# WarmCongee/SDUMC

Hardware: AMD Instinct MI355X
Metric: train samples/sec at MOSEI feature shapes (two-stream forward + 6-term loss + backward + Adam) (higher is better)
Workload: dtype f32

## Files before the change

sdumc_amd/csrc/chain_cluster.hip:

```cpp
#include <atomic>
#include <mutex>

#include "chain_common.h"

namespace {

constexpr int CL = 4;
constexpr int OC = D / CL;
constexpr int HC = H / CL;
constexpr int PARTC = NWV * 7 * OC;
constexpr int SPIN_CAP = 400000;
static_assert(PARTC >= NWV * 2 * H, "tail layers");

template <int R> using FwdA = FwdALds<R, PARTC>;
template <int R> using FwdB = FwdBLds<R, PARTC, 3, 0>;
template <int R> using BwdB = BwdBLds<R, PARTC, 3>;
template <int R> using BwdA = BwdALds<R, PARTC, 3>;

struct Cl {
  uint32_t* arrive;
  uint32_t* depart;
  int32_t* err;
  uint32_t round;
  bool hold;
// ... 17 lines not shown
  for (int u = threadIdx.x; u < ROWS * q; u += NTHR) {
    const int r = u / q, c = u - r * q;
    st4(dst_lds + r * ld_dst + 4 * c, row0 + r < nrows ? ld4_dev(src + (int64_t)(row0 + r) * ld_src + 4 * c) : f32x4{0.f, 0.f, 0.f, 0.f});
  }
}

__device__ __forceinline__ void cl_sync(Cl& cl, int* s_bail) {
  if (cl.mode & 1u) __builtin_amdgcn_fence(__ATOMIC_RELEASE, "agent");
  __builtin_amdgcn_s_waitcnt(0);
  __syncthreads();
  if (threadIdx.x == 0 && !*s_bail) {
    if (!cl.hold) {
      if (cl.mode & 1u) __hip_atomic_fetch_add(cl.arrive, 1u, __ATOMIC_RELEASE, __HIP_MEMORY_SCOPE_AGENT);
      else __hip_atomic_fetch_add(cl.arrive, 1u, __ATOMIC_RELAXED, __HIP_MEMORY_SCOPE_AGENT);
    }
    const uint32_t want = (uint32_t)CL * (cl.round + 1u);
    int spins = 0;
    while (__hip_atomic_load(cl.arrive, __ATOMIC_RELAXED, __HIP_MEMORY_SCOPE_AGENT) < want) {
      if (++spins > SPIN_CAP) {
        *s_bail = 1;
        __hip_atomic_store(cl.err, 1, __ATOMIC_RELAXED, __HIP_MEMORY_SCOPE_AGENT);
        break;
      }
      __builtin_amdgcn_s_sleep(1);
    }
  }
  ++cl.round;
  __syncthreads();
  if (cl.mode & 1u) __builtin_amdgcn_fence(__ATOMIC_ACQUIRE, "agent");
}
__device__ __forceinline__ void cl_exit(Cl& cl) {
  if (threadIdx.x == 0) {
    const uint32_t n = __hip_atomic_fetch_add(cl.depart, 1u, __ATOMIC_RELAXED, __HIP_MEMORY_SCOPE_AGENT);
    if (n == (uint32_t)CL - 1u) {
      __hip_atomic_store(cl.arrive, 0u, __ATOMIC_RELAXED, __HIP_MEMORY_SCOPE_AGENT);
      __hip_atomic_store(cl.depart, 0u, __ATOMIC_RELAXED, __HIP_MEMORY_SCOPE_AGENT);
    }
  }
}

template <int I, int O, int RSv>
struct CGeom {
  static constexpr int OG = O / 4;
  static constexpr int S = 64 / OG;
  static constexpr int MW = NWV / RSv;
  static constexpr int UNITS = I / (4 * S);
  static constexpr int WAVES = UNITS >= MW ? MW : UNITS;
  static constexpr int IW = I / WAVES;
  static constexpr int ITER = IW / (4 * S);
  static constexpr int PRE = ITER >= 4 ? 4 : ITER;
  static_assert(O == 32 || O == 64, "slice width");
  static_assert(I % (4 * S * WAVES) == 0 && ITER >= 1, "k range must split evenly");
};
struct CRing {
  uint4 w[16];
};
template <int N, class F>
__device__ __forceinline__ void static_for(F&& f) {
  if constexpr (N > 0) {
    static_for<N - 1>(f);
    f(std::integral_constant<int, N - 1>{});
  }
}

template <int I, int O, int RSv, int SLOT>
__device__ __forceinline__ void cxm_load(CRing& ring, const float* mp, int j, int ldm) {
  using G = CGeom<I, O, RSv>;
  static_for<4>([&](auto ec) {
    constexpr int e = decltype(ec)::value;
    ring.w[SLOT * 4 + e] = *reinterpret_cast<const uint4*>(mp + (size_t)(j * 4 * G::S + e) * ldm);
  });
}

template <int I, int O, int RSv>
__device__ __forceinline__ void cxm_prefetch(CRing& ring, const float* __restrict__ M, int ldm) {
  using G = CGeom<I, O, RSv>;
  const int lane = threadIdx.x & 63, wg = (threadIdx.x >> 6) % G::MW;
  if (wg < G::WAVES) {
    const int sq = lane / G::OG, cg = lane % G::OG;
    const float* mp = M + (size_t)(wg * G::IW + 4 * sq) * ldm + 4 * cg;
    static_for<G::PRE>([&](auto dc) { cxm_load<I, O, RSv, decltype(dc)::value>(ring, mp, decltype(dc)::value, ldm); });
    static_for<16 - 4 * G::PRE>([&](auto kc) { ring.w[4 * G::PRE + decltype(kc)::value] = uint4{0u, 0u, 0u, 0u}; });
  }
}

template <int I, int O, int RSv>
__device__ __forceinline__ void cxm_selfcheck(const CRing& ring, const float* M, int ldm, uint32_t* dbg) {
  using G = CGeom<I, O, RSv>;
  const int lane = threadIdx.x & 63, wg = (threadIdx.x >> 6) % G::MW;
  if (wg < G::WAVES && dbg) {
    const int sq = lane / G::OG, cg = lane % G::OG;
    const float* mp = M + (size_t)(wg * G::IW + 4 * sq) * ldm + 4 * cg;
    static_for<G::PRE>([&](auto dc) {
      constexpr int sl = decltype(dc)::value;
      static_for<4>([&](auto ec) {
        constexpr int e = decltype(ec)::value;
        const uint32_t* ad = reinterpret_cast<const uint32_t*>(mp + (size_t)(sl * 4 * G::S + e) * ldm);
        const uint4 c = ring.w[sl * 4 + e];
        uint32_t b[4];
#pragma unroll
        for (int k = 0; k < 4; ++k) b[k] = __hip_atomic_load(ad + k, __ATOMIC_RELAXED, __HIP_MEMORY_SCOPE_AGENT);
        if (c.x != b[0] || c.y != b[1] || c.z != b[2] || c.w != b[3]) {
          const uint32_t idx = atomicAdd(dbg, 1u);
          if (idx < 20) {
            uint32_t* r = dbg + 8 + 12 * idx;
            r[0] = blockIdx.x; r[1] = threadIdx.x; r[2] = sl * 4 + e;
            r[3] = (uint32_t)(reinterpret_cast<uintptr_t>(ad) & 0xffffffffu);
            r[4] = c.x; r[5] = c.y; r[6] = c.z; r[7] = c.w; r[8] = b[0]; r[9] = b[1]; r[10] = b[2]; r[11] = b[3];
          }
        }
      });
    });
  }
}

constexpr int FOLD_MAXCHUNK = 32;
template <class T>
__device__ __forceinline__ T sel3v(T t0, T t1, T t2, int m) { return m == 0 ? t0 : (m == 1 ? t1 : t2); }
#define sel3(t, m) sel3v((t)[0], (t)[1], (t)[2], m)

struct ChunkItem {
  const float* src;
  int u, c0, nc;
};
template <int NU, class Desc>
__device__ __forceinline__ ChunkItem chunk_item(int u, int c0, Desc& desc) {
  ChunkItem it;
  it.u = u;
  it.c0 = c0;
  desc(min(u, NU - 1), it.src, it.nc);
  if (u >= NU) it.nc = -1;
  return it;
}
template <int STRIDE>
__device__ __forceinline__ void chunk_request(const ChunkItem& it, f32x4 (&pv)[8]) {
  static_for<8>([&](auto jc) {
    constexpr int j = decltype(jc)::value;
    if (it.c0 + j < it.nc) pv[j] = ld4(it.src + (size_t)(it.c0 + j) * STRIDE);
  });
}
template <int NU, int STRIDE, class Desc, class Acc, class Fin>
__device__ __forceinline__ void chunk_drain(ChunkItem cur, f32x4 (&pa)[8], Desc& desc, Acc&& acc, Fin&& fin) {
  f32x4 sum = {0.f, 0.f, 0.f, 0.f};
  while (cur.nc >= 0) {
    const bool more = cur.c0 + 8 < cur.nc;
    const ChunkItem nx = chunk_item<NU>(more ? cur.u : cur.u + NTHR, more ? cur.c0 + 8 : 0, desc);
    f32x4 pb[8];
    chunk_request<STRIDE>(nx, pb);
    if (cur.c0 == 0) sum = f32x4{0.f, 0.f, 0.f, 0.f};
    static_for<8>([&](auto jc) {
      constexpr int j = decltype(jc)::value;
      if (cur.c0 + j < cur.nc) acc(sum, pa[j], cur.u, cur.c0 + j);
    });
    if (!more) fin(cur.u, sum);
    cur = nx;
    static_for<8>([&](auto jc) { pa[decltype(jc)::value] = pb[decltype(jc)::value]; });
  }
}

template <int R, int NQT>
struct FoldHead {
  static constexpr int NS = 3 * R * NQT;
  static constexpr int NU = NS * (D / 4);
  static_assert(NS <= NTHR, "one statistics row per thread");
  float cm[8], cs[8];
  ChunkItem it;
// ... 154 lines not shown
}

template <int ROWS>
__device__ __forceinline__ void lds_selfcheck(const float* lds_rows, const float* src, int width, int row0, int nrows, uint32_t* dbg, int tag) {
  if (!dbg) return;
  const int q = width >> 2;
  for (int u = threadIdx.x; u < ROWS * q; u += NTHR) {
    const int r = u / q, c = u - r * q;
    if (row0 + r >= nrows) continue;
    const f32x4 l = ld4(lds_rows + r * width + 4 * c);
    const f32x4 g = ld4(src + (int64_t)(row0 + r) * width + 4 * c);
    if (__float_as_uint(l[0]) != __float_as_uint(g[0]) || __float_as_uint(l[1]) != __float_as_uint(g[1]) ||
        __float_as_uint(l[2]) != __float_as_uint(g[2]) || __float_as_uint(l[3]) != __float_as_uint(g[3])) {
      const uint32_t idx = atomicAdd(dbg, 1u);
      if (idx < 20) {
        uint32_t* rec = dbg + 8 + 12 * idx;
        rec[0] = blockIdx.x; rec[1] = threadIdx.x; rec[2] = (uint32_t)tag; rec[3] = (uint32_t)(r * width + 4 * c);
#pragma unroll
        for (int k = 0; k < 4; ++k) { rec[4 + k] = __float_as_uint(l[k]); rec[8 + k] = __float_as_uint(g[k]); }
      }
    }
  }
}

template <int ROWS, int I, int O, class Epi, class Hook>
__device__ __forceinline__ void cxm_run(CRing& ring, const float* in_lds, int ld_in, const float* __restrict__ M, int ldm, float* part,
                                        Epi&& epi, Hook&& hook) {
  constexpr int RSv = ROWS >= 14 ? 2 : 1;
  using G = CGeom<I, O, RSv>;
  constexpr int OG = G::OG, S = G::S, MW = G::MW, WAVES = G::WAVES, IW = G::IW, ITER = G::ITER;
  constexpr int RG = ROWS / RSv;
  static_assert(ROWS % RSv == 0 && RG <= 7, "rows per group");
  static_assert(RSv * WAVES * RG * O <= PARTC, "partial-sum area too small");
  const int tid = threadIdx.x, lane = tid & 63, wave = tid >> 6;
  const int grp = wave / MW, wg = wave % MW;
  const int sq = lane / OG, cg = lane % OG;
  f32x4 acc[RG];
#pragma unroll
  for (int r = 0; r < RG; ++r) acc[r] = f32x4{0.f, 0.f, 0.f, 0.f};
  if (wg < WAVES) {
    const int i0 = wg * IW + 4 * sq;
    const float* mp = M + (size_t)i0 * ldm + 4 * cg;
    const float* xin = in_lds + grp * RG * ld_in + i0;
    static_for<ITER>([&](auto jc) {
      constexpr int j = decltype(jc)::value, sl = (j % 4) * 4;
#pragma unroll
      for (int r = 0; r < RG; ++r) {
        const f32x4 x = ld4(xin + r * ld_in + j * 4 * S);
        static_for<4>([&](auto ec) {
          constexpr int e = decltype(ec)::value;
          const uint4 u = ring.w[sl + e];
          acc[r] += f32x4{__uint_as_float(u.x), __uint_as_float(u.y), __uint_as_float(u.z), __uint_as_float(u.w)} * x[e];
        });
      }
      __builtin_amdgcn_sched_barrier(0);
      if constexpr (j + 4 < ITER) cxm_load<I, O, RSv, j % 4>(ring, mp, j + 4, ldm);
    });
#pragma unroll
    for (int r = 0; r < RG; ++r)
#pragma unroll
      for (int c = 0; c < 4; ++c) {
        acc[r][c] += __shfl_xor(acc[r][c], 32, 64);
        acc[r][c] += __shfl_xor(acc[r][c], 16, 64);
        if constexpr (S == 8) acc[r][c] += __shfl_xor(acc[r][c], 8, 64);
      }
  }
  hook();
  if (wg < WAVES && sq == 0) {
#pragma unroll
    for (int r = 0; r < RG; ++r) st4(part + ((grp * WAVES + wg) * RG + r) * O + 4 * cg, acc[r]);
  }
  __syncthreads();
  for (int u = tid; u < ROWS * (O / 4); u += NTHR) {
    const int r = u / (O / 4), cq = u - r * (O / 4);
    const int g = r / RG, rr = r - g * RG;
    f32x4 v = ld4(part + ((g * WAVES) * RG + rr) * O + 4 * cq);
#pragma unroll
    for (int ww = 1; ww < WAVES; ++ww) v += ld4(part + ((g * WAVES + ww) * RG + rr) * O + 4 * cq);
    epi(r, 4 * cq, v);
  }
  __syncthreads();
}

#define TR(k) do { if (a.cl_trace && blockIdx.x == 0 && threadIdx.x == 0) a.cl_trace[k] = wall_clock64(); } while (0)

#define CL_PROLOGUE()                                                                                          \
  __shared__ int s_bail;                                                                                       \
  const int cluster = blockIdx.x % ncl, member = blockIdx.x / ncl;                                             \
  const int V = a.V, v0 = cluster * R, tid = threadIdx.x, lane = tid & 63, wave = tid >> 6;                    \
  const int coff = member * OC;                                                                                \
  Cl cl{a.cl_flags + cluster * 64, a.cl_flags + cluster * 64 + 32, a.cl_err, 0u, a.cl_test_hold == 1 && blockIdx.x == 0, (uint32_t)a.cl_mode};                              \
  if (tid == 0) s_bail = 0;                                                                                    \
  (void)lane; (void)wave

typedef float WT;
#define PF(I_, O_, ptr, ldm) cxm_prefetch<I_, O_, 1>(ring, ptr, ldm)
#define PF14(I_, O_, ptr, ldm) cxm_prefetch<I_, O_, 2>(ring, ptr, ldm)

template <int R>
__device__ __forceinline__ void chain_fwd_a_cl_body(const sdumc_chain_args a, const int ncl) {
  extern __shared__ __attribute__((aligned(16))) float sm[];
  using L = FwdA<R>;
  float *part = sm + L::part, *s_hpre = sm + L::hpre, *s_u1 = sm + L::u1, *s_u = sm + L::u, *s_att1 = sm + L::att1, *s_att2 = sm + L::att2,
        *s_qin = sm + L::qin, *s_q = sm + L::q, *s_bias = sm + L::bias;
  CL_PROLOGUE();
  TR(0);
  const int64_t VD = (int64_t)V * D;
  const bool fold = a.fra.part[0] != nullptr;
  FoldHead<R, 1> fh;
  FoldNorm<R, 1> fn;
  if (fold) {
    fold_request<R, 1>(fh, a.fra, v0, V);
    fold_norm_request<R, 1>(fn, a.fra, v0, V, member);
  }
  constexpr int NBIAS = (FWD_A_BIAS_UNITS + NTHR - 1) / NTHR;
  f32x4 bias[NBIAS];
  static_for<NBIAS>([&](auto kc) { bias[decltype(kc)::value] = ld4(fwd_a_bias_src(a, min(tid + decltype(kc)::value * NTHR, FWD_A_BIAS_UNITS - 1))); });
  const DropRT dbase = drop_resolve(a.drop);
  CRing ring;
  if (a.cl_mode & 2) __builtin_amdgcn_fence(__ATOMIC_ACQUIRE, "agent");
  if (a.cl_mode & 8)
    for (int i = 0; i < 8; ++i) __builtin_amdgcn_s_sleep(127);
  PF(D, OC, a.umlp0_w[0] + coff, D);
  if (a.cl_mode & 16) cxm_selfcheck<D, OC, 1>(ring, a.umlp0_w[0] + coff, D, a.cl_dbg);
  if (fold) fold_combine<R, 1>(fh, a.fra, a.hpre, s_hpre, s_qin, v0, V, member, dbase);
  else for (int m = 0; m < 3; ++m) load_rows<R>(s_hpre + m * R * D, a.hpre + m * VD, D, D, v0, V);
  static_for<NBIAS>([&](auto kc) {
    const int u = tid + decltype(kc)::value * NTHR;
    if (u < FWD_A_BIAS_UNITS) st4(s_bias + 4 * u, bias[decltype(kc)::value]);
  });
  __syncthreads();
  TR(11);
  if ((a.cl_mode & 64) && !a.fra.part[0])
    for (int m = 0; m < 3; ++m) lds_selfcheck<R>(s_hpre + m * R * D, a.hpre + m * VD, D, v0, V, a.cl_dbg, 10 + m);
#pragma unroll 1
  for (int m = 0; m < 3; ++m) {
    const DropRT dr = mkdrop_rt(dbase, 6 + 2 * m, 1, D);
    float* dst = a.u1 + m * VD + (int64_t)v0 * D;
    auto epi = [&](int r, int col, f32x4 v) {
      col += coff;
      if (v0 + r < V) st4_dev(dst + (int64_t)r * D + col, fwd_val(v, s_bias + m * D, col, true, dr, (uint32_t)(v0 + r)));
    };
    cxm_run<R, D, OC>(ring, s_hpre + m * R * D, D, a.umlp0_w[m] + coff, D, part, epi,
                                [&] { PF(D, OC, (m < 2 ? a.umlp0_w[m + 1] : a.umlp3_w[0]) + coff, D); });
  }
  if (fold) fold_norm_finish<R, 1>(fn, a.fra, s_qin, v0, V, member);
  TR(1);
  if ((a.cl_mode & 64) && !a.fra.part[0])
    for (int m = 0; m < 3; ++m) lds_selfcheck<R>(s_hpre + m * R * D, a.hpre + m * VD, D, v0, V, a.cl_dbg, 20 + m);
  cl_sync(cl, &s_bail);
  TR(2);
  for (int m = 0; m < 3; ++m) reload_rows<R>(s_u1 + m * R * D, D, a.u1 + m * VD, D, D, v0, V);
  __syncthreads();
#pragma unroll 1
  for (int m = 0; m < 3; ++m) {
    const DropRT dr = mkdrop_rt(dbase, 7 + 2 * m, 1, D);
    float* dst = a.u + (int64_t)v0 * 3 * D + m * D;
    auto epi = [&](int r, int col, f32x4 v) {
      col += coff;
      if (v0 + r < V) st4_dev(dst + (int64_t)r * 3 * D + col, fwd_val(v, s_bias + (3 + m) * D, col, true, dr, (uint32_t)(v0 + r)));
    };
    cxm_run<R, D, OC>(ring, s_u1 + m * R * D, D, a.umlp3_w[m] + coff, D, part, epi, [&] {
      if (m < 2) PF(D, OC, a.umlp3_w[m + 1] + coff, D);
      else PF(3 * D, OC, a.att0_w + coff, D);
    });
  }
  TR(3);
  cl_sync(cl, &s_bail);
  TR(4);
  reload_rows<R>(s_u, 3 * D, a.u, 3 * D, 3 * D, v0, V);
  __syncthreads();
  {
    const DropRT dr = mkdrop_rt(dbase, 12, 1, D);
    float* dst = a.att1 + (int64_t)v0 * D;
    auto epi = [&](int r, int col, f32x4 v) {
      col += coff;
      if (v0 + r < V) st4_dev(dst + (int64_t)r * D + col, fwd_val(v, s_bias + 6 * D, col, true, dr, (uint32_t)(v0 + r)));
    };
    cxm_run<R, 3 * D, OC>(ring, s_u, 3 * D, a.att0_w + coff, D, part, epi, [&] { PF(D, OC, a.att3_w + coff, D); });
  }
  TR(5);
  cl_sync(cl, &s_bail);
  TR(6);
  reload_rows<R>(s_att1, D, a.att1, D, D, v0, V);
  __syncthreads();
  {
    const DropRT dr = mkdrop_rt(dbase, 13, 1, D);
    float* dst = a.att2 + (int64_t)v0 * D;
    auto epi = [&](int r, int col, f32x4 v) {
      col += coff;
      if (v0 + r < V) st4_dev(dst + (int64_t)r * D + col, fwd_val(v, s_bias + 7 * D, col, true, dr, (uint32_t)(v0 + r)));
    };
    cxm_run<R, D, OC>(ring, s_att1, D, a.att3_w + coff, D, part, epi, [&] { PF(D, OC, a.query_w[0] + coff, D); });
  }
  TR(7);
  cl_sync(cl, &s_bail);
  TR(8);
  reload_rows<R>(s_att2, D, a.att2, D, D, v0, V);
  __syncthreads();
  fwd_a_alpha<L>(a, sm, v0, V, member == 0);
  fwd_a_fusion<L>(a, sm, v0, V, [member](int c) { return c / OC == member; });
#pragma unroll 1
  for (int i = 0; i < 7; ++i) {
    const DropRT dr = mkdrop_rt(dbase, 14 + i, 1, D);
    float* dst = a.q + (int64_t)v0 * NQ * D + i * D;
    float* th = (i == 5 && a.o_text_hidden) ? a.o_text_hidden + (int64_t)v0 * D : nullptr;
    auto epi = [&](int r, int col, f32x4 v) {
      col += coff;
      if (v0 + r < V) {
        const f32x4 y = fwd_val(v, s_bias + (8 + i) * D, col, true, dr, (uint32_t)(v0 + r));
        st4_dev(dst + (int64_t)r * NQ * D + col, y);
        if (th) st4(th + (int64_t)r * D + col, y);
      }
    };
    cxm_run<R, D, OC>(ring, s_qin + i * R * D, D, a.query_w[i] + coff, D, part, epi,
                                [&] { if (i < 6) PF(D, OC, a.query_w[i + 1] + coff, D); else PF14(D, OC, a.caq_w[0] + coff, D); });
  }
  TR(9);
  cl_sync(cl, &s_bail);
  TR(10);
  reload_rows<R>(s_q, NQ * D, a.q, NQ * D, NQ * D, v0, V);
  __syncthreads();
  cl_exit(cl);
#pragma unroll 1
  for (int m = 0; m < 3; ++m) {
    float* dst = a.qp + ((int64_t)m * V + v0) * NQ * D;
    auto epi = [&](int r, int col, f32x4 v) {
      col += coff;
      if (v0 + r / NQ < V) st4(dst + (int64_t)r * D + col, v + ld4(s_bias + (15 + m) * D + col));
    };
    cxm_run<NQ * R, D, OC>(ring, s_q, D, a.caq_w[m] + coff, D, part, epi, [&] { if (m < 2) PF14(D, OC, a.caq_w[m + 1] + coff, D); });
  }
  TR(31);
}
template <int R>
__global__ __launch_bounds__(NTHR) void chain_fwd_a_cl_kernel(const sdumc_chain_args a, const int ncl) { chain_fwd_a_cl_body<R>(a, ncl); }

template <int R>
__device__ __forceinline__ void chain_fwd_b_cl_body(const sdumc_chain_args a, const int ncl) {
  extern __shared__ __attribute__((aligned(16))) float sm[];
  using L = FwdB<R>;
  float *part = sm + L::part, *s_x = sm + L::x, *s_c = sm + L::c, *s_h = sm + L::h, *s_e1 = sm + L::e1, *s_e2 = sm + L::e2, *s_bias = sm + L::bias;
  CL_PROLOGUE();
  TR(0);
  const int64_t VQ = (int64_t)V * NQ;
  const int hoff = member * HC;
  const bool fold = a.ca.part[0] != nullptr;
  FoldHead<R, NQ> fh;
  FoldNorm<R, NQ> fn;
  if (fold) {
    fold_request<R, NQ>(fh, a.ca, v0, V);
    fold_norm_request<R, NQ>(fn, a.ca, v0, V, member);
  }
  static_assert(FWD_B_BIAS_UNITS <= NTHR, "one bias unit per thread");
  const f32x4 bias = ld4(fwd_b_bias_src(a, min(tid, FWD_B_BIAS_UNITS - 1)));
  const float al = alpha_request<R>(a.alpha, v0, V);
  const DropRT dbase = drop_resolve(a.drop);
  CRing ring;
  PF14(D, OC, a.cmlp0_w[0] + coff, D);
  if (fold) fold_combine<R, NQ>(fh, a.ca, a.ca_out, s_x, s_c, v0, V, member, dbase);
  else for (int m = 0; m < 3; ++m) load_rows<NQ * R>(s_x + m * NQ * R * D, a.ca_out + (int64_t)m * VQ * D, D, D, v0 * NQ, V * NQ);
  if (tid < FWD_B_BIAS_UNITS) st4(s_bias + 4 * tid, bias);
  alpha_store<R>(al, sm + L::alpha, v0, V);
  __syncthreads();
  TR(11);
#pragma unroll 1
  for (int m = 0; m < 3; ++m) {
    const DropRT dr = mkdrop_rt(dbase, 27 + 2 * m, NQ, D);
    float* dst = a.c1 + ((int64_t)m * VQ + (int64_t)v0 * NQ) * D;
    auto epi = [&](int r, int col, f32x4 v) {
      col += coff;
      if (v0 * NQ + r < V * NQ) st4_dev(dst + (int64_t)r * D + col, fwd_val(v, s_bias + m * D, col, true, dr, (uint32_t)(v0 * NQ + r)));
    };
    cxm_run<NQ * R, D, OC>(ring, s_x + m * NQ * R * D, D, a.cmlp0_w[m] + coff, D, part, epi, [&] {
      if (m < 2) PF14(D, OC, a.cmlp0_w[m + 1] + coff, D);
      else PF14(D, HC, a.cmlp3_w[0] + hoff, H);
    });
  }
  if (fold) fold_norm_finish<R, NQ>(fn, a.ca, s_c, v0, V, member);
  TR(1);
  cl_sync(cl, &s_bail);
  TR(2);
  for (int m = 0; m < 3; ++m) reload_rows<NQ * R>(s_x + m * NQ * R * D, D, a.c1 + (int64_t)m * VQ * D, D, D, v0 * NQ, V * NQ);
  __syncthreads();
#pragma unroll 1
  for (int m = 0; m < 3; ++m) {
    const DropRT dr = mkdrop_rt(dbase, 28 + 2 * m, NQ, H);
    float* dst = a.c + ((int64_t)m * VQ + (int64_t)v0 * NQ) * H;
    float* ct = (m == 1 && a.o_cross_text) ? a.o_cross_text + (int64_t)v0 * NQ * H : nullptr;
    auto epi = [&](int r, int col, f32x4 v) {
      col += hoff;
      if (v0 * NQ + r < V * NQ) {
        const f32x4 y = fwd_val(v, s_bias + 3 * D + m * H, col, true, dr, (uint32_t)(v0 * NQ + r));
        st4_dev(dst + (int64_t)r * H + col, y);
        if (ct) st4(ct + (int64_t)r * H + col, y);
      }
    };
    cxm_run<NQ * R, D, HC>(ring, s_x + m * NQ * R * D, D, a.cmlp3_w[m] + hoff, H, part, epi, [&] {
      if (m < 2) PF14(D, HC, a.cmlp3_w[m + 1] + hoff, H);
// ... 132 lines not shown
                                     [&] { if (m < 2) PF14(D, OC, a.cmlp0_w[m + 1] + coff, D); });
  }
  TR(31);
}
template <int R>
__global__ __launch_bounds__(NTHR) void chain_bwd_b_cl_kernel(const sdumc_chain_args a, const int ncl) { chain_bwd_b_cl_body<R>(a, ncl); }

template <int R>
__device__ __forceinline__ void chain_bwd_a_cl_body(const sdumc_chain_args a, const int ncl) {
  extern __shared__ __attribute__((aligned(16))) float sm[];
  using L = BwdA<R>;
  float *part = sm + L::part, *s_x = sm + L::x, *s_dq = sm + L::dq, *s_dqin = sm + L::dqin, *s_u = sm + L::u, *s_du = sm + L::du, *s_a2 = sm + L::a2,
        *s_a1 = sm + L::a1, *s_u1 = sm + L::u1;
  CL_PROLOGUE();
  TR(0);
  const int64_t VD = (int64_t)V * D, VQ = (int64_t)V * NQ;
  const float sc = a.relu_scale;
  const bool wr = member == 0;

  const bool slabs = a.dq_part[0] != nullptr;
  auto dq_desc = [&](int u, const float*& src, int& nc) {
    const int row = u / (D / 4), cq = u - row * (D / 4);
    const int mr = row / NQ, i = row - mr * NQ;
    const int m = mr / R, v = v0 + (mr - m * R);
    const int ncm = sel3(a.dq_nchunk, m);
    src = sel3(a.dq_part, m) + ((size_t)min(v, V - 1) * ncm * NQ + i) * D + 4 * cq;
    nc = v < V ? ncm : 0;
  };
  constexpr int NUX = 3 * R * NQ * (D / 4);
  ChunkItem it;
  f32x4 pa[8];
  RowsReg<NQ * R, D> x[3];
  if (slabs) {
    it = chunk_item<NUX>(tid, 0, dq_desc);
    chunk_request<NQ * D>(it, pa);
  } else {
    static_for<3>([&](auto mc) { rows_request(x[decltype(mc)::value], a.d_qp + (int64_t)decltype(mc)::value * VQ * D, D, v0 * NQ, V * NQ); });
  }
  const float al = alpha_request<R>(a.alpha, v0, V), dal = alpha_request<R>(a.d_alpha, v0, V);
  CRing ring;
  PF14(D, OC, a.caq_w[0] + coff, D);
  RowsReg<R, 3 * D> g_u;
  RowsReg<R, D> g_a2, g_a1, g_u1[3];
  rows_request(g_u, a.u, 3 * D, v0, V);
  rows_request(g_a2, a.att2, D, v0, V);
  rows_request(g_a1, a.att1, D, v0, V);
  static_for<3>([&](auto mc) { rows_request(g_u1[decltype(mc)::value], a.u1 + decltype(mc)::value * VD, D, v0, V); });
  if (slabs) {
    chunk_drain<NUX, NQ * D>(
        it, pa, dq_desc, [](f32x4& sum, const f32x4 pv, int, int) { sum += pv; },
        [&](int u, const f32x4 sum) {
          const int row = u / (D / 4), cq = u - row * (D / 4);
          const int mr = row / NQ, i = row - mr * NQ;
          const int m = mr / R, v = v0 + (mr - m * R);
          if (v < V && (mr & (CL - 1)) == member) st4(a.d_qp + (((size_t)m * V + v) * NQ + i) * D + 4 * cq, sum);
          st4(s_x + (size_t)row * D + 4 * cq, sum);
        });
  } else {
    static_for<3>([&](auto mc) { rows_store(x[decltype(mc)::value], s_x + decltype(mc)::value * NQ * R * D, v0 * NQ, V * NQ); });
  }
  alpha_store<R>(al, sm + L::alpha, v0, V);
  alpha_store<R>(dal, sm + L::dalpha, v0, V);
  __syncthreads();
#pragma unroll 1
  for (int m = 0; m < 3; ++m) {
    auto epi = [&](int r, int col, f32x4 v) {
      col += coff;
      if (m > 0) v += ld4(s_dq + r * D + col);
      st4(s_dq + r * D + col, v);
    };
    cxm_run<NQ * R, D, OC>(ring, s_x + m * NQ * R * D, D, a.caq_w[m] + coff, D, part, epi,
                                     [&] { if (m < 2) PF14(D, OC, a.caq_w[m + 1] + coff, D); else PF(D, OC, a.query_w[0] + coff, D); });
  }
  bwd_a_mask_q<L, OC>(a, sm, v0, V, sc, coff, [](f32x4 g, float*, float* hbm, bool live) {
    if (live) st4_dev(hbm, g);
  });
  rows_store(g_u, s_u, v0, V);
  rows_store(g_a2, s_a2, v0, V);
  rows_store(g_a1, s_a1, v0, V);
  static_for<3>([&](auto mc) { rows_store(g_u1[decltype(mc)::value], s_u1 + decltype(mc)::value * R * D, v0, V); });
  TR(1);
  cl_sync(cl, &s_bail);
  TR(2);
  reload_rows<R>(s_dq, NQ * D, a.d_q, NQ * D, NQ * D, v0, V);
  __syncthreads();
#pragma unroll 1
  for (int i = 0; i < 7; ++i) {
    float* dst = a.d_qin + i * VD + (int64_t)v0 * D;
    auto epi = [&](int r, int col, f32x4 v) {
      col += coff;
      if (v0 + r < V) st4_dev(dst + (int64_t)r * D + col, v);
    };
    cxm_run<R, D, OC>(ring, s_dq + i * D, NQ * D, a.query_w[i] + coff, D, part, epi,
                                [&] { PF(D, OC, (i < 6 ? a.query_w[i + 1] : a.att3_w) + coff, D); });
  }
  TR(3);
  cl_sync(cl, &s_bail);
  TR(4);
  for (int i = 0; i < 7; ++i) reload_rows<R>(s_dqin + i * R * D, D, a.d_qin + i * VD, D, D, v0, V);
  __syncthreads();
  bwd_a_fusion<L>(a, sm, v0, V, wr);
  bwd_a_datt2<L>(a, sm, v0, V, sc, wr);
  {
    float* dst = a.d_att1 + (int64_t)v0 * D;
    auto epi = [&](int r, int col, f32x4 v) {
      col += coff;
      if (v0 + r < V) st4_dev(dst + (int64_t)r * D + col, mask_val(v, ld4(s_a1 + r * D + col), sc));
    };
    cxm_run<R, D, OC>(ring, s_a2, D, a.att3_w + coff, D, part, epi, [&] { PF(D, OC, a.att0_w + member * OC, 3 * D); });
  }
  TR(5);
  cl_sync(cl, &s_bail);
  TR(6);
  reload_rows<R>(s_a1, D, a.d_att1, D, D, v0, V);
  __syncthreads();
#pragma unroll 1
  for (int blk = member; blk < 12; blk += CL) {
    float* dst = a.d_u + (int64_t)v0 * 3 * D;
    const int boff = blk * OC;
    auto epi = [&](int r, int col, f32x4 v) {
      col += boff;
      if (v0 + r < V) st4_dev(dst + (int64_t)r * 3 * D + col, mask_val(v + ld4(s_du + r * 3 * D + col), ld4(s_u + r * 3 * D + col), sc));
    };
    cxm_run<R, D, OC>(ring, s_a1, D, a.att0_w + boff, 3 * D, part, epi, [&] {
      if (blk + CL < 12) PF(D, OC, a.att0_w + boff + CL * OC, 3 * D);
      else PF(D, OC, a.umlp3_w[0] + coff, D);
    });
  }
  TR(7);
  cl_sync(cl, &s_bail);
  TR(8);
  reload_rows<R>(s_du, 3 * D, a.d_u, 3 * D, 3 * D, v0, V);
  __syncthreads();
#pragma unroll 1
  for (int m = 0; m < 3; ++m) {
    float* dst = a.d_u1 + m * VD + (int64_t)v0 * D;
    const float* y = s_u1 + m * R * D;
    auto epi = [&](int r, int col, f32x4 v) {
      col += coff;
      if (v0 + r < V) st4_dev(dst + (int64_t)r * D + col, mask_val(v, ld4(y + r * D + col), sc));
    };
    cxm_run<R, D, OC>(ring, s_du + m * D, 3 * D, a.umlp3_w[m] + coff, D, part, epi,
                                [&] { PF(D, OC, (m < 2 ? a.umlp3_w[m + 1] : a.umlp0_w[0]) + coff, D); });
  }
  TR(9);
  cl_sync(cl, &s_bail);
  TR(10);
  cl_exit(cl);
  for (int m = 0; m < 3; ++m) reload_rows<R>(s_u1 + m * R * D, D, a.d_u1 + m * VD, D, D, v0, V);
  __syncthreads();
#pragma unroll 1
  for (int m = 0; m < 3; ++m) {
    float* dst = a.d_hpre + m * VD + (int64_t)v0 * D;
    auto epi = [&](int r, int col, f32x4 v) {
      col += coff;
      if (v0 + r < V) st4(dst + (int64_t)r * D + col, v);
    };
    cxm_run<R, D, OC>(ring, s_u1 + m * R * D, D, a.umlp0_w[m] + coff, D, part, epi,
                                [&] { if (m < 2) PF(D, OC, a.umlp0_w[m + 1] + coff, D); });
  }
  TR(31);
}
template <int R>
__global__ __launch_bounds__(NTHR) void chain_bwd_a_cl_kernel(const sdumc_chain_args a, const int ncl) { chain_bwd_a_cl_body<R>(a, ncl); }

#undef PF
#undef PF14
#undef CL_PROLOGUE

struct ClusterDev {
  std::mutex mu;
  uint32_t* flags = nullptr;
  int32_t* err = nullptr;
  unsigned long long* trace = nullptr;
  uint32_t* dbg = nullptr;
  bool tracing = false;
  hipEvent_t done = nullptr;
  hipStream_t last = nullptr;
  bool any = false;
  bool multi = false;
  int cus = 0;
  int attr = 0;
  int test_hold = 0;
};
ClusterDev g_cl[16];
constexpr int kMaxClusters = 128;

ClusterDev* cluster_dev() {
  int dev = 0;
  if (hipGetDevice(&dev) != hipSuccess || dev < 0 || dev >= 16) return nullptr;
  ClusterDev& d = g_cl[dev];
  std::lock_guard<std::mutex> lk(d.mu);
  if (!d.flags) {
    int cus = 0;
    if (hipDeviceGetAttribute(&cus, hipDeviceAttributeMultiprocessorCount, dev) != hipSuccess) return nullptr;
    uint32_t* f = nullptr;
    if (hipMalloc(&f, (kMaxClusters * 64 + 64 + 256 + 256) * sizeof(uint32_t)) != hipSuccess) return nullptr;
    if (hipMemset(f, 0, (kMaxClusters * 64 + 64 + 256 + 256) * sizeof(uint32_t)) != hipSuccess) return nullptr;
    d.trace = reinterpret_cast<unsigned long long*>(f + kMaxClusters * 64 + 64);
    d.dbg = f + kMaxClusters * 64 + 64 + 256;
    if (hipEventCreateWithFlags(&d.done, hipEventDisableTiming) != hipSuccess) return nullptr;
    d.err = reinterpret_cast<int32_t*>(f + kMaxClusters * 64);
    d.cus = cus;
    d.flags = f;
  }
  return &d;
}

}

namespace { std::atomic<int> g_cluster_on{-1}; }
extern "C" int sdumc_set_chain_cluster(int on) {
  g_cluster_on.store(on ? 1 : 0);
  return SDUMC_OK;
}
namespace {
template <int R>
bool cluster_prepare(ClusterDev* d) {
  std::lock_guard<std::mutex> lk(d->mu);
  if (d->attr == 0) {
    d->attr = -1;
    if (!(sdumc_set_dyn_lds(chain_fwd_a_cl_kernel<R>, 158 * 1024) && sdumc_set_dyn_lds(chain_fwd_b_cl_kernel<R>, FwdB<R>::bytes) &&
          sdumc_set_dyn_lds(chain_bwd_b_cl_kernel<R>, BwdB<R>::bytes) && sdumc_set_dyn_lds(chain_bwd_a_cl_kernel<R>, BwdA<R>::bytes)))
      return false;
    int n[4] = {0, 0, 0, 0};
    if (hipOccupancyMaxActiveBlocksPerMultiprocessor(&n[0], chain_fwd_a_cl_kernel<R>, NTHR, FwdA<R>::bytes) != hipSuccess ||
        hipOccupancyMaxActiveBlocksPerMultiprocessor(&n[1], chain_fwd_b_cl_kernel<R>, NTHR, FwdB<R>::bytes) != hipSuccess ||
        hipOccupancyMaxActiveBlocksPerMultiprocessor(&n[2], chain_bwd_b_cl_kernel<R>, NTHR, BwdB<R>::bytes) != hipSuccess ||
        hipOccupancyMaxActiveBlocksPerMultiprocessor(&n[3], chain_bwd_a_cl_kernel<R>, NTHR, BwdA<R>::bytes) != hipSuccess)
      return false;
    if (n[0] < 1 || n[1] < 1 || n[2] < 1 || n[3] < 1) return false;
    d->attr = 1;
  }
  return d->attr == 1;
}
}

extern "C" int sdumc_chain_cluster_ok_(int V) {
  if (g_cluster_on.load() < 0) { const char* e = getenv("SDUMC_CHAIN_CLUSTER"); g_cluster_on.store(e ? (atoi(e) ? 1 : 0) : 1); }
  if (!g_cluster_on.load()) return 0;
  return sdumc_chain_cluster_fits_(V);
}
extern "C" int sdumc_chain_cluster_fits_(int V) {
  if (V <= 0) return 0;
  ClusterDev* d = cluster_dev();
  if (!d) return 0;
  const int ncl = (V + 1) / 2;
  if (!(ncl <= kMaxClusters && ncl * CL <= d->cus)) return 0;
  return cluster_prepare<2>(d) ? 1 : 0;
}
// ... 138 lines not shown
```

sdumc_amd/csrc/engine.hip:

```cpp
#include <stdio.h>
#include <string.h>

#include <algorithm>
#include <atomic>
#include <map>
#include <cstdlib>
#include <cstring>
#include <mutex>
#include <string>
#include <tuple>
#include <vector>

#include "common.h"

extern "C" int sdumc_axpy2d(const float* src, int32_t ld_src, float* dst, int32_t ld_dst, int32_t rows, int32_t cols,
                            void* stream);

namespace {

constexpr int D = SDUMC_D, H = SDUMC_H, NQ = SDUMC_NQ, RD = SDUMC_RNC_DIM;

constexpr int SITE_IN[2][3] = {{0, 2, 4}, {21, 23, 25}};
constexpr int SITE_OUT[2][3] = {{1, 3, 5}, {22, 24, 26}};
constexpr int SITE_UMLP0 = 6, SITE_UMLP1 = 7;
// ... 2649 lines not shown
  sdumc_net_grads g;
  memset(&g, 0, sizeof(g));
  g.d_vals = dout;
  g.d_fused = dout + 64 * V;
  g.d_rnc = g.d_fused + H * V;
  g.d_text_hidden = g.d_rnc + RD * V;
  g.d_cross_text = g.d_text_hidden + D * V;
  g.grads = reinterpret_cast<float*>(base + sl.grads);
  const SplitScope split_scope(&nio);
  Ctx bc{*d, nio, as_stream(stream), build_params(d->da, d->dt, d->dv), Plan(), nullptr, nullptr, nullptr};
  RET(ctx_init(bc));
  bc.G = g.grads;
  const BwdSchedule sch = plan_backward(bc, 3);
  RET(sch.rc);
  mark(static_cast<hipStream_t>(stream), 0);
  RET(net_forward_impl(d, &nio, stream, false));
  bool total_pending = false;
  RET(loss_backward_impl(d, &nio, cfg, &g, base + sl.loss, sl.net - sl.loss, stream, cfg->hyper, &total_pending));
  mark(static_cast<hipStream_t>(stream), 5);
  RET(backward(bc, g, sch));
  mark(static_cast<hipStream_t>(stream), 9);
  sdumc_total_loss tl;
  tl.losses = cfg->losses;
  tl.chain_err = sdumc_chain_cluster_err_ptr_();
  for (int i = 0; i < 6; ++i) tl.w[i] = cfg->weights[i];
  RET(sdumc_adam_apply_(io->params, g.grads, cfg->adam_m, cfg->adam_v, (int64_t)sl.live, cfg->hyper, cfg->beta1, cfg->beta2,
                        cfg->eps, cfg->weight_decay, 1.0f, d->train ? const_cast<uint32_t*>(io->rng_state) : nullptr, 2u,
                        total_pending ? &tl : nullptr, stream));
  mark(static_cast<hipStream_t>(stream), 10);
  return SDUMC_OK;
}

extern "C" int sdumc_debug_marks(int on) {
  g_marks_on = on != 0;
  return SDUMC_OK;
}
extern "C" int sdumc_debug_marks_read(float* ms, int n) {
  for (int i = 0; i < n; ++i) {
    ms[i] = -1.f;
    if (i < kMarks && g_mark_set[i] && g_mark_set[0]) {
      float t = 0.f;
      if (hipEventElapsedTime(&t, g_marks[0], g_marks[i]) == hipSuccess) ms[i] = t;
    }
  }
  return SDUMC_OK;
}

extern "C" int32_t sdumc_debug_plan_table(const sdumc_net_dims* d, char* buf, size_t buflen) {
  Plan p;
  if (!d || !make_plan(*d, p)) return 0;
  const int HS = p.hf ? 2 : 1;
  const int64_t V = p.V;
  std::string s;
  auto put = [&](const std::string& name, int64_t off, int64_t n) {
    char line[160];
    snprintf(line, sizeof(line), "%s %lld %lld\n", name.c_str(), (long long)off, (long long)n);
    s += line;
  };
  const char* mod[3] = {"a", "t", "v"};
  for (int m = 0; m < 3; ++m) {
    put(std::string("x_") + mod[m], p.x[m][0], p.rows[m] / (m == 1 ? 1 : p.S) * D / HS);
    for (int k = 0; k < 2; ++k) {
      const std::string sfx = std::to_string(k) + mod[m];
      put("keys" + sfx, p.keys[k][m], p.rows[m] * D / HS);
      put("attn" + sfx, p.attn[k][m], p.rows[m] * (k == 0 ? 1 : NQ));
      put("pooled" + sfx, p.pooled[k][m], V * (k == 0 ? 1 : NQ) * D);
    }
  }
  put("hpre", p.hpre, 3 * V * D); put("u1", p.u1, 3 * V * D); put("u", p.u, 3 * V * D); put("att1", p.att1, V * D);
  put("att2", p.att2, V * D); put("alpha", p.alpha, V * 3); put("qin", p.qin, 7 * V * D); put("q", p.q, 7 * V * D);
  put("qp", p.qp, 3 * V * NQ * D); put("ca_out", p.ca_out, 3 * V * NQ * D); put("c1", p.c1, 3 * V * NQ * D);
  put("c", p.c, 3 * V * NQ * H); put("h", p.h, V * NQ * H); put("e1", p.e1, V * D); put("e2", p.e2, V * H);
  put("beta", p.beta, V * NQ); put("z", p.z, V * H); put("vals", p.vals, V); put("r1", p.r1, V * RD); put("r", p.r, V * RD);
  put("wt", p.wt, build_params(d->da, d->dt, d->dv).early);
  for (int m = 0; m < 3; ++m) {
    for (int k = 0; k < 2; ++k) {
      const std::string sfx = std::to_string(k) + mod[m];
      put("dz" + sfx, p.dz[k][m], p.rows[m] * D / HS);
      if (p.dom[k][m]) put("dom" + sfx, p.dom[k][m], V * (k == 0 ? 1 : NQ) * D);
    }
    put(std::string("dx_") + mod[m], p.dx[m][0], p.rows[m] / (m == 1 ? 1 : p.S) * D / HS);
  }
  put("d_hpre", p.d_hpre, 3 * V * D); put("d_ca_out", p.d_ca_out, 3 * V * NQ * D);
  if (!buf || s.size() + 1 > buflen) return -(int32_t)(s.size() + 1);
  memcpy(buf, s.c_str(), s.size() + 1);
  return (int32_t)s.size();
}

extern "C" int sdumc_plan_attn_layout_(const sdumc_net_dims* d, sdumc_attn_layout* out) {
  Plan p;
  if (!d || !out || !make_plan(*d, p)) return SDUMC_EINVAL;
  out->B = p.B;
  out->S = p.S;
  for (int m = 0; m < 3; ++m)
    for (int s = 0; s < 2; ++s) out->T[m][s] = p.T[m][s];
  for (int k = 0; k < 2; ++k)
    for (int m = 0; m < 3; ++m) out->attn[k][m] = p.attn[k][m];
  out->total = p.cur;
  return SDUMC_OK;
}

extern "C" size_t sdumc_step_grads_offset(const sdumc_net_dims* d) {
  if (!d || d->streams != 2) return 0;
  return step_layout(*d).grads;
}
```

Before: 51270.

## Group consecutive small cluster GEMM layers with a double-buffered weight ring and one reduction

Adds cxm_group_run, which runs two or three independent 2-row layers back to back. Each layer's weights fill half of the register ring, so the next layer's weights load into the other half while the current one computes. The per-wave partial-sum write, the __syncthreads and the cross-wave reduction are each done once per group instead of once per layer. The forward and backward umlp, query and att0 sequences in the clustered chain kernels now use this path, with prefetch of the upper ring half (PFH). It also exports more debug buffers (d_u1, d_u, d_qin, d_h, d_c) from the engine. The cost is higher register and partial-sum LDS pressure, plus more template instantiations.

```diff
diff --git a/sdumc_amd/csrc/chain_cluster.hip b/sdumc_amd/csrc/chain_cluster.hip
--- a/sdumc_amd/csrc/chain_cluster.hip
+++ b/sdumc_amd/csrc/chain_cluster.hip
@@ -123,6 +123,16 @@
     static_for<G::PRE>([&](auto dc) { cxm_load<I, O, RSv, decltype(dc)::value>(ring, mp, decltype(dc)::value, ldm); });
     static_for<16 - 4 * G::PRE>([&](auto kc) { ring.w[4 * G::PRE + decltype(kc)::value] = uint4{0u, 0u, 0u, 0u}; });
   }
+}
+
+template <int I, int O>
+__device__ __forceinline__ void cxm_prefetch_hi(CRing& ring, const float* __restrict__ M1, int ldm) {
+  using G = CGeom<I, O, 1>;
+  static_assert(G::ITER == 2 && G::WAVES == G::MW, "a layer is half of the ring, on every wave");
+  const int lane = threadIdx.x & 63, wg = threadIdx.x >> 6;
+  const int sq = lane / G::OG, cg = lane % G::OG;
+  const size_t off = (size_t)(wg * G::IW + 4 * sq) * ldm + 4 * cg;
+  static_for<2>([&](auto jc) { cxm_load<I, O, 1, 2 + decltype(jc)::value>(ring, M1 + off, decltype(jc)::value, ldm); });
 }
 
 template <int I, int O, int RSv>
@@ -443,6 +453,67 @@
   __syncthreads();
 }
 
+template <int NG, int ROWS, int I, int O, class In, class Mat, class Epi, class Hook>
+__device__ __forceinline__ void cxm_group_run(CRing& ring, In&& in, int ld_in, Mat&& mat, int ldm, float* part, Epi&& epi, Hook&& hook) {
+  using G = CGeom<I, O, 1>;
+  constexpr int OG = G::OG, S = G::S, WAVES = G::WAVES, IW = G::IW, ITER = G::ITER;
+  constexpr int LP = WAVES * ROWS * O;
+  static_assert(ROWS < 14 && ITER == 2 && WAVES == G::MW, "2-row layers that fill half of the ring, on every wave");
+  static_assert(NG >= 2 && NG <= NWV && NG * LP <= PARTC, "partial-sum area too small");
+  static_assert(ROWS * (O / 4) <= 64, "one wave finishes a layer");
+  const int tid = threadIdx.x, lane = tid & 63, wg = tid >> 6;
+  const int sq = lane / OG, cg = lane % OG;
+  const int i0 = wg * IW + 4 * sq;
+  static_for<NG>([&](auto gc) {
+    constexpr int g = decltype(gc)::value, h = (g % 2) * ITER;
+    const float* xin = in(gc) + i0;
+    f32x4 acc[ROWS];
+#pragma unroll
+    for (int r = 0; r < ROWS; ++r) acc[r] = f32x4{0.f, 0.f, 0.f, 0.f};
+    static_for<ITER>([&](auto jc) {
+      constexpr int j = decltype(jc)::value, sl = (h + j) * 4;
+#pragma unroll
+      for (int r = 0; r < ROWS; ++r) {
+        const f32x4 x = ld4(xin + r * ld_in + j * 4 * S);
+        static_for<4>([&](auto ec) {
+          constexpr int e = decltype(ec)::value;
+          const uint4 u = ring.w[sl + e];
+          acc[r] += f32x4{__uint_as_float(u.x), __uint_as_float(u.y), __uint_as_float(u.z), __uint_as_float(u.w)} * x[e];
+        });
+      }
+      __builtin_amdgcn_sched_barrier(0);
+    });
+    if constexpr (g + 2 < NG) {
+      const float* mn = mat(std::integral_constant<int, g + 2>{}) + (size_t)i0 * ldm + 4 * cg;
+      static_for<ITER>([&](auto jc) { cxm_load<I, O, 1, h + decltype(jc)::value>(ring, mn, decltype(jc)::value, ldm); });
+    }
+    if constexpr (g + 1 == NG) hook();
+#pragma unroll
+    for (int r = 0; r < ROWS; ++r)
+#pragma unroll
+      for (int c = 0; c < 4; ++c) {
+        acc[r][c] += __shfl_xor(acc[r][c], 32, 64);
+        acc[r][c] += __shfl_xor(acc[r][c], 16, 64);
+        if constexpr (S == 8) acc[r][c] += __shfl_xor(acc[r][c], 8, 64);
+      }
+    if (sq == 0) {
+#pragma unroll
+      for (int r = 0; r < ROWS; ++r) st4(part + g * LP + (wg * ROWS + r) * O + 4 * cg, acc[r]);
+    }
+  });
+  __syncthreads();
+  if (wg < NG && lane < ROWS * (O / 4)) {
+    const int g = __builtin_amdgcn_readfirstlane(wg);
+    const int r = lane / (O / 4), cq = lane - r * (O / 4);
+    const float* pl = part + g * LP + r * O + 4 * cq;
+    f32x4 v = ld4(pl);
+#pragma unroll
+    for (int ww = 1; ww < WAVES; ++ww) v += ld4(pl + ww * ROWS * O);
+    epi(g, r, 4 * cq, v);
+  }
+  __syncthreads();
+}
+
 #define TR(k) do { if (a.cl_trace && blockIdx.x == 0 && threadIdx.x == 0) a.cl_trace[k] = wall_clock64(); } while (0)
 
 #define CL_PROLOGUE()                                                                                          \
@@ -457,6 +528,7 @@
 typedef float WT;
 #define PF(I_, O_, ptr, ldm) cxm_prefetch<I_, O_, 1>(ring, ptr, ldm)
 #define PF14(I_, O_, ptr, ldm) cxm_prefetch<I_, O_, 2>(ring, ptr, ldm)
+#define PFH(I_, O_, ptr, ldm) cxm_prefetch_hi<I_, O_>(ring, ptr, ldm)
 
 template <int R>
 __device__ __forceinline__ void chain_fwd_a_cl_body(const sdumc_chain_args a, const int ncl) {
@@ -486,6 +558,7 @@
   if (a.cl_mode & 16) cxm_selfcheck<D, OC, 1>(ring, a.umlp0_w[0] + coff, D, a.cl_dbg);
   if (fold) fold_combine<R, 1>(fh, a.fra, a.hpre, s_hpre, s_qin, v0, V, member, dbase);
   else for (int m = 0; m < 3; ++m) load_rows<R>(s_hpre + m * R * D, a.hpre + m * VD, D, D, v0, V);
+  PFH(D, OC, a.umlp0_w[1] + coff, D);
   static_for<NBIAS>([&](auto kc) {
     const int u = tid + decltype(kc)::value * NTHR;
     if (u < FWD_A_BIAS_UNITS) st4(s_bias + 4 * u, bias[decltype(kc)::value]);
@@ -494,16 +567,15 @@
   TR(11);
   if ((a.cl_mode & 64) && !a.fra.part[0])
     for (int m = 0; m < 3; ++m) lds_selfcheck<R>(s_hpre + m * R * D, a.hpre + m * VD, D, v0, V, a.cl_dbg, 10 + m);
-#pragma unroll 1
-  for (int m = 0; m < 3; ++m) {
-    const DropRT dr = mkdrop_rt(dbase, 6 + 2 * m, 1, D);
-    float* dst = a.u1 + m * VD + (int64_t)v0 * D;
-    auto epi = [&](int r, int col, f32x4 v) {
-      col += coff;
+  {
+    auto epi = [&](int m, int r, int col, f32x4 v) {
+      col += coff;
+      const DropRT dr = mkdrop_rt(dbase, 6 + 2 * m, 1, D);
+      float* dst = a.u1 + m * VD + (int64_t)v0 * D;
       if (v0 + r < V) st4_dev(dst + (int64_t)r * D + col, fwd_val(v, s_bias + m * D, col, true, dr, (uint32_t)(v0 + r)));
     };
-    cxm_run<R, D, OC>(ring, s_hpre + m * R * D, D, a.umlp0_w[m] + coff, D, part, epi,
-                                [&] { PF(D, OC, (m < 2 ? a.umlp0_w[m + 1] : a.umlp3_w[0]) + coff, D); });
+    cxm_group_run<3, R, D, OC>(ring, [&](auto m) { return s_hpre + m * R * D; }, D, [&](auto m) { return a.umlp0_w[m] + coff; }, D, part, epi,
+                               [&] { PF(D, OC, a.umlp3_w[0] + coff, D); });
   }
   if (fold) fold_norm_finish<R, 1>(fn, a.fra, s_qin, v0, V, member);
   TR(1);
@@ -511,20 +583,18 @@
     for (int m = 0; m < 3; ++m) lds_selfcheck<R>(s_hpre + m * R * D, a.hpre + m * VD, D, v0, V, a.cl_dbg, 20 + m);
   cl_sync(cl, &s_bail);
   TR(2);
+  PFH(D, OC, a.umlp3_w[1] + coff, D);
   for (int m = 0; m < 3; ++m) reload_rows<R>(s_u1 + m * R * D, D, a.u1 + m * VD, D, D, v0, V);
   __syncthreads();
-#pragma unroll 1
-  for (int m = 0; m < 3; ++m) {
-    const DropRT dr = mkdrop_rt(dbase, 7 + 2 * m, 1, D);
-    float* dst = a.u + (int64_t)v0 * 3 * D + m * D;
-    auto epi = [&](int r, int col, f32x4 v) {
-      col += coff;
+  {
+    auto epi = [&](int m, int r, int col, f32x4 v) {
+      col += coff;
+      const DropRT dr = mkdrop_rt(dbase, 7 + 2 * m, 1, D);
+      float* dst = a.u + (int64_t)v0 * 3 * D + m * D;
       if (v0 + r < V) st4_dev(dst + (int64_t)r * 3 * D + col, fwd_val(v, s_bias + (3 + m) * D, col, true, dr, (uint32_t)(v0 + r)));
     };
-    cxm_run<R, D, OC>(ring, s_u1 + m * R * D, D, a.umlp3_w[m] + coff, D, part, epi, [&] {
-      if (m < 2) PF(D, OC, a.umlp3_w[m + 1] + coff, D);
-      else PF(3 * D, OC, a.att0_w + coff, D);
-    });
+    cxm_group_run<3, R, D, OC>(ring, [&](auto m) { return s_u1 + m * R * D; }, D, [&](auto m) { return a.umlp3_w[m] + coff; }, D, part, epi,
+                               [&] { PF(3 * D, OC, a.att0_w + coff, D); });
   }
   TR(3);
   cl_sync(cl, &s_bail);
@@ -557,25 +627,35 @@
   TR(7);
   cl_sync(cl, &s_bail);
   TR(8);
+  PFH(D, OC, a.query_w[1] + coff, D);
   reload_rows<R>(s_att2, D, a.att2, D, D, v0, V);
   __syncthreads();
   fwd_a_alpha<L>(a, sm, v0, V, member == 0);
   fwd_a_fusion<L>(a, sm, v0, V, [member](int c) { return c / OC == member; });
-#pragma unroll 1
-  for (int i = 0; i < 7; ++i) {
-    const DropRT dr = mkdrop_rt(dbase, 14 + i, 1, D);
-    float* dst = a.q + (int64_t)v0 * NQ * D + i * D;
-    float* th = (i == 5 && a.o_text_hidden) ? a.o_text_hidden + (int64_t)v0 * D : nullptr;
-    auto epi = [&](int r, int col, f32x4 v) {
-      col += coff;
-      if (v0 + r < V) {
-        const f32x4 y = fwd_val(v, s_bias + (8 + i) * D, col, true, dr, (uint32_t)(v0 + r));
-        st4_dev(dst + (int64_t)r * NQ * D + col, y);
-        if (th) st4(th + (int64_t)r * D + col, y);
-      }
-    };
-    cxm_run<R, D, OC>(ring, s_qin + i * R * D, D, a.query_w[i] + coff, D, part, epi,
-                                [&] { if (i < 6) PF(D, OC, a.query_w[i + 1] + coff, D); else PF14(D, OC, a.caq_w[0] + coff, D); });
+  {
+    auto query_group = [&](auto nc, auto ic, auto&& hook) {
+      constexpr int N = decltype(nc)::value, I0 = decltype(ic)::value;
+      auto epi = [&](int g, int r, int col, f32x4 v) {
+        col += coff;
+        const int i = I0 + g;
+        const DropRT dr = mkdrop_rt(dbase, 14 + i, 1, D);
+        float* dst = a.q + (int64_t)v0 * NQ * D + i * D;
+        float* th = (i == 5 && a.o_text_hidden) ? a.o_text_hidden + (int64_t)v0 * D : nullptr;
+        if (v0 + r < V) {
+          const f32x4 y = fwd_val(v, s_bias + (8 + i) * D, col, true, dr, (uint32_t)(v0 + r));
+          st4_dev(dst + (int64_t)r * NQ * D + col, y);
+          if (th) st4(th + (int64_t)r * D + col, y);
+        }
+      };
+      cxm_group_run<N, R, D, OC>(ring, [&](auto g) { return s_qin + (I0 + g) * R * D; }, D, [&](auto g) { return a.query_w[I0 + g] + coff; }, D,
+                                 part, epi, hook);
+    };
+    using std::integral_constant;
+    query_group(integral_constant<int, 3>{}, integral_constant<int, 0>{}, [&] { PF(D, OC, a.query_w[3] + coff, D); });
+    PFH(D, OC, a.query_w[4] + coff, D);
+    query_group(integral_constant<int, 2>{}, integral_constant<int, 3>{}, [&] { PF(D, OC, a.query_w[5] + coff, D); });
+    PFH(D, OC, a.query_w[6] + coff, D);
+    query_group(integral_constant<int, 2>{}, integral_constant<int, 5>{}, [&] { PF14(D, OC, a.caq_w[0] + coff, D); });
   }
   TR(9);
   cl_sync(cl, &s_bail);
@@ -874,17 +954,26 @@
   TR(1);
   cl_sync(cl, &s_bail);
   TR(2);
+  PFH(D, OC, a.query_w[1] + coff, D);
   reload_rows<R>(s_dq, NQ * D, a.d_q, NQ * D, NQ * D, v0, V);
   __syncthreads();
-#pragma unroll 1
-  for (int i = 0; i < 7; ++i) {
-    float* dst = a.d_qin + i * VD + (int64_t)v0 * D;
-    auto epi = [&](int r, int col, f32x4 v) {
-      col += coff;
-      if (v0 + r < V) st4_dev(dst + (int64_t)r * D + col, v);
-    };
-    cxm_run<R, D, OC>(ring, s_dq + i * D, NQ * D, a.query_w[i] + coff, D, part, epi,
-                                [&] { PF(D, OC, (i < 6 ? a.query_w[i + 1] : a.att3_w) + coff, D); });
+  {
+    auto query_group = [&](auto nc, auto ic, auto&& hook) {
+      constexpr int N = decltype(nc)::value, I0 = decltype(ic)::value;
+      auto epi = [&](int g, int r, int col, f32x4 v) {
+        col += coff;
+        float* dst = a.d_qin + (I0 + g) * VD + (int64_t)v0 * D;
+        if (v0 + r < V) st4_dev(dst + (int64_t)r * D + col, v);
+      };
+      cxm_group_run<N, R, D, OC>(ring, [&](auto g) { return s_dq + (I0 + g) * D; }, NQ * D, [&](auto g) { return a.query_w[I0 + g] + coff; }, D,
+                                 part, epi, hook);
+    };
+    using std::integral_constant;
+    query_group(integral_constant<int, 3>{}, integral_constant<int, 0>{}, [&] { PF(D, OC, a.query_w[3] + coff, D); });
+    PFH(D, OC, a.query_w[4] + coff, D);
+    query_group(integral_constant<int, 2>{}, integral_constant<int, 3>{}, [&] { PF(D, OC, a.query_w[5] + coff, D); });
+    PFH(D, OC, a.query_w[6] + coff, D);
+    query_group(integral_constant<int, 2>{}, integral_constant<int, 5>{}, [&] { PF(D, OC, a.att3_w + coff, D); });
   }
   TR(3);
   cl_sync(cl, &s_bail);
@@ -904,52 +993,48 @@
   TR(5);
   cl_sync(cl, &s_bail);
   TR(6);
+  PFH(D, OC, a.att0_w + (member + CL) * OC, 3 * D);
   reload_rows<R>(s_a1, D, a.d_att1, D, D, v0, V);
   __syncthreads();
-#pragma unroll 1
-  for (int blk = member; blk < 12; blk += CL) {
-    float* dst = a.d_u + (int64_t)v0 * 3 * D;
-    const int boff = blk * OC;
-    auto epi = [&](int r, int col, f32x4 v) {
-      col += boff;
+  {
+    auto epi = [&](int g, int r, int col, f32x4 v) {
+      float* dst = a.d_u + (int64_t)v0 * 3 * D;
+      col += (member + g * CL) * OC;
       if (v0 + r < V) st4_dev(dst + (int64_t)r * 3 * D + col, mask_val(v + ld4(s_du + r * 3 * D + col), ld4(s_u + r * 3 * D + col), sc));
     };
-    cxm_run<R, D, OC>(ring, s_a1, D, a.att0_w + boff, 3 * D, part, epi, [&] {
-      if (blk + CL < 12) PF(D, OC, a.att0_w + boff + CL * OC, 3 * D);
-      else PF(D, OC, a.umlp3_w[0] + coff, D);
-    });
+    cxm_group_run<3, R, D, OC>(ring, [&](auto) { return s_a1; }, D, [&](auto g) { return a.att0_w + (member + g * CL) * OC; }, 3 * D, part, epi,
+                               [&] { PF(D, OC, a.umlp3_w[0] + coff, D); });
   }
   TR(7);
   cl_sync(cl, &s_bail);
   TR(8);
+  PFH(D, OC, a.umlp3_w[1] + coff, D);
   reload_rows<R>(s_du, 3 * D, a.d_u, 3 * D, 3 * D, v0, V);
   __syncthreads();
-#pragma unroll 1
-  for (int m = 0; m < 3; ++m) {
-    float* dst = a.d_u1 + m * VD + (int64_t)v0 * D;
-    const float* y = s_u1 + m * R * D;
-    auto epi = [&](int r, int col, f32x4 v) {
-      col += coff;
+  {
+    auto epi = [&](int m, int r, int col, f32x4 v) {
+      col += coff;
+      float* dst = a.d_u1 + m * VD + (int64_t)v0 * D;
+      const float* y = s_u1 + m * R * D;
       if (v0 + r < V) st4_dev(dst + (int64_t)r * D + col, mask_val(v, ld4(y + r * D + col), sc));
     };
-    cxm_run<R, D, OC>(ring, s_du + m * D, 3 * D, a.umlp3_w[m] + coff, D, part, epi,
-                                [&] { PF(D, OC, (m < 2 ? a.umlp3_w[m + 1] : a.umlp0_w[0]) + coff, D); });
+    cxm_group_run<3, R, D, OC>(ring, [&](auto m) { return s_du + m * D; }, 3 * D, [&](auto m) { return a.umlp3_w[m] + coff; }, D, part, epi,
+                               [&] { PF(D, OC, a.umlp0_w[0] + coff, D); });
   }
   TR(9);
   cl_sync(cl, &s_bail);
   TR(10);
   cl_exit(cl);
+  PFH(D, OC, a.umlp0_w[1] + coff, D);
   for (int m = 0; m < 3; ++m) reload_rows<R>(s_u1 + m * R * D, D, a.d_u1 + m * VD, D, D, v0, V);
   __syncthreads();
-#pragma unroll 1
-  for (int m = 0; m < 3; ++m) {
-    float* dst = a.d_hpre + m * VD + (int64_t)v0 * D;
-    auto epi = [&](int r, int col, f32x4 v) {
-      col += coff;
+  {
+    auto epi = [&](int m, int r, int col, f32x4 v) {
+      col += coff;
+      float* dst = a.d_hpre + m * VD + (int64_t)v0 * D;
       if (v0 + r < V) st4(dst + (int64_t)r * D + col, v);
     };
-    cxm_run<R, D, OC>(ring, s_u1 + m * R * D, D, a.umlp0_w[m] + coff, D, part, epi,
-                                [&] { if (m < 2) PF(D, OC, a.umlp0_w[m + 1] + coff, D); });
+    cxm_group_run<3, R, D, OC>(ring, [&](auto m) { return s_u1 + m * R * D; }, D, [&](auto m) { return a.umlp0_w[m] + coff; }, D, part, epi, [] {});
   }
   TR(31);
 }
@@ -958,6 +1043,7 @@
 
 #undef PF
 #undef PF14
+#undef PFH
 #undef CL_PROLOGUE
 
 struct ClusterDev {
diff --git a/sdumc_amd/csrc/engine.hip b/sdumc_amd/csrc/engine.hip
--- a/sdumc_amd/csrc/engine.hip
+++ b/sdumc_amd/csrc/engine.hip
@@ -2755,6 +2755,8 @@
     put(std::string("dx_") + mod[m], p.dx[m][0], p.rows[m] / (m == 1 ? 1 : p.S) * D / HS);
   }
   put("d_hpre", p.d_hpre, 3 * V * D); put("d_ca_out", p.d_ca_out, 3 * V * NQ * D);
+  put("d_u1", p.d_u1, 3 * V * D); put("d_u", p.d_u, 3 * V * D); put("d_qin", p.d_qin, 7 * V * D); put("d_h", p.d_h, V * NQ * H);
+  put("d_c", p.d_c, 3 * V * NQ * H);
   if (!buf || s.size() + 1 > buflen) return -(int32_t)(s.size() + 1);
   memcpy(buf, s.c_str(), s.size() + 1);
   return (int32_t)s.size();
```

Result: no change. 51470 (median of 6 runs) (+0.4%).
